# OmarZOS/deep-learning-at-scale

Measured on AMD Instinct MI355X. Metric: rows/sec (whole node), LSTM seq64 regression at 1/2/4/8 MI355X; val MSE parity, higher is better.
Workload: dtype bf16; 1 GPU; global_batch=8192, per_gpu_batch=8192, seq_len=64, parallelism=dp1

## Files before the change

deep-learning-at-scale_amd/csrc/binding.cpp:

```cpp
#include <torch/extension.h>
#include <ATen/hip/impl/HIPStreamMasqueradingAsCUDA.h>
#include <ATen/hip/impl/HIPGuardImplMasqueradingAsCUDA.h>

#include <cstdlib>
#include <map>
#include <type_traits>
#include <mutex>
#include <vector>

#include "kernels.h"

namespace {

using wf::bf16_t;

int diag_env(const char* name, int dflt) {
  if (wf::dbg_mask() != ~0) return dflt;
  const char* v = std::getenv(name);
  return v != nullptr ? std::atoi(v) : dflt;
}

bool disable_glds() {
  static const bool off = diag_env("WELLFLOW_NO_GLDS", 0) == 1;
  return off;
}

hipStream_t cur_stream() { return c10::hip::getCurrentHIPStreamMasqueradingAsCUDA().stream(); }

void check_t(const at::Tensor& t, at::ScalarType dt, const char* name) {
  TORCH_CHECK(t.defined(), name, ": undefined tensor");
  TORCH_CHECK(t.is_cuda(), name, ": must be a GPU tensor");
  TORCH_CHECK(t.scalar_type() == dt, name, ": expected dtype ", dt, " got ", t.scalar_type());
  TORCH_CHECK(t.is_contiguous(), name, ": must be contiguous");
  TORCH_CHECK(reinterpret_cast<uintptr_t>(t.data_ptr()) % 16 == 0, name,
              ": data pointer must be 16-byte aligned");
}

void check_extent(const at::Tensor& t, int64_t need, const char* name) {
  TORCH_CHECK(t.numel() >= need, name, ": needs at least ", need, " elements, has ", t.numel());
}

bf16_t* bfp(const at::Tensor& t) { return reinterpret_cast<bf16_t*>(t.data_ptr()); }
float* fp(const at::Tensor& t) { return t.data_ptr<float>(); }

template <class T>
T* opt_ptr(const c10::optional<at::Tensor>& t, at::ScalarType dt, const char* name,
           int64_t need) {
  if (!t.has_value() || !t->defined()) return nullptr;
  check_t(*t, dt, name);
  check_extent(*t, need, name);
  return reinterpret_cast<T*>(t->data_ptr());
}

int64_t operand_extent(bool mn, int64_t rows, int64_t K, int64_t ld) {
  if (rows == 0 || K == 0) return 0;
  return mn ? (K - 1) * ld + rows : (rows - 1) * ld + K;
}

void gemm(const at::Tensor& A, bool a_mn, int64_t lda, const at::Tensor& B, bool b_mn, int64_t ldb,
          int64_t M, int64_t N, int64_t K, int64_t ksplit, c10::optional<at::Tensor> outF,
          c10::optional<at::Tensor> outH, int64_t ldo, c10::optional<at::Tensor> bias,
          c10::optional<at::Tensor> mask, int64_t ldm, double mask_scale,
          c10::optional<at::Tensor> colsum, double alpha, double beta, int64_t act, bool atomic,
          double drop_p, int64_t seed, int64_t big_tile, c10::optional<at::Tensor> seed_dev) {
  TORCH_CHECK(wf::dw_tile_valid(big_tile), "gemm: tile ", big_tile, " does not exist; valid ids are 0 (128x128), ",
              "1 (256x128), 3 (256x192), 4 / 5 (256x192, 5- / 4-slot ring), 7 (best for N)");
  check_t(A, at::kBFloat16, "A");
  check_t(B, at::kBFloat16, "B");
  TORCH_CHECK(M > 0 && N > 0 && K > 0, "gemm: empty problem");
  TORCH_CHECK(lda % 8 == 0 && ldb % 8 == 0, "gemm: lda/ldb must be multiples of 8");
  TORCH_CHECK(a_mn ? (M % 8 == 0) : (K % 8 == 0), "gemm: A contiguous extent must be a multiple of 8");
  TORCH_CHECK(b_mn ? (N % 8 == 0) : (K % 8 == 0), "gemm: B contiguous extent must be a multiple of 8");
  TORCH_CHECK(a_mn ? lda >= M : lda >= K, "gemm: lda too small");
  TORCH_CHECK(b_mn ? ldb >= N : ldb >= K, "gemm: ldb too small");
  check_extent(A, operand_extent(a_mn, M, K, lda), "A");
  check_extent(B, operand_extent(b_mn, N, K, ldb), "B");
  TORCH_CHECK(ldo >= N, "gemm: ldo < N");
  const int64_t out_need = (M - 1) * ldo + N;
  wf::GemmEpilogue e;
  e.outF = opt_ptr<float>(outF, at::kFloat, "outF", out_need);
  e.outH = opt_ptr<bf16_t>(outH, at::kBFloat16, "outH", out_need);
  TORCH_CHECK(e.outF || e.outH, "gemm: need an output");
  TORCH_CHECK(!atomic || (e.outF && !e.outH && beta == 0.0), "gemm: atomic needs outF only, beta 0");
  TORCH_CHECK(beta == 0.0 || e.outF, "gemm: beta needs outF");
  e.ldo = ldo;
  e.bias = opt_ptr<float>(bias, at::kFloat, "bias", N);
  if (mask.has_value() && mask->defined()) TORCH_CHECK(ldm >= N, "gemm: ldm < N");
  e.mask = opt_ptr<bf16_t>(mask, at::kBFloat16, "mask", (M - 1) * ldm + N);
  e.ldm = ldm;
  e.mask_scale = (float)mask_scale;
  e.colsum = opt_ptr<float>(colsum, at::kFloat, "colsum", N);
  e.alpha = (float)alpha;
  e.beta = (float)beta;
  e.act = (int)act;
  e.atomic = atomic ? 1 : 0;
  e.drop_p = (float)drop_p;
  e.seed = (unsigned long long)seed;
  if (seed_dev.has_value() && seed_dev->defined()) {
    TORCH_CHECK(seed_dev->is_cuda() && seed_dev->scalar_type() == at::kLong && seed_dev->numel() >= 1,
                "gemm: seed_dev must be a GPU int64 tensor");
    e.seed_dev = reinterpret_cast<const long long*>(seed_dev->data_ptr<int64_t>());
  }
  e.big_tile = (int)big_tile;
  TORCH_CHECK(ksplit == 1 || atomic, "gemm: split-K needs atomic accumulation");
  e.stage_ok = (e.outH != nullptr && e.outF == nullptr && !atomic && beta == 0.0 && N % 8 == 0 &&
                ldo % 8 == 0 && (e.mask == nullptr || ldm % 8 == 0))
                   ? 1 : 0;
  const int64_t Mc = (M + 127) / 128 * 128, Nc = (N + 127) / 128 * 128;
  int64_t kchunk = (K + std::max<int64_t>(ksplit, 1) - 1) / std::max<int64_t>(ksplit, 1);
  kchunk = (kchunk + 63) / 64 * 64;
  const bool glds_ok = (K % 64 == 0) && (kchunk % 64 == 0) &&
                       A.numel() >= operand_extent(a_mn, Mc, K, lda) + (a_mn ? 0 : 0) &&
                       B.numel() >= operand_extent(b_mn, Nc, K, ldb) &&
                       (a_mn || Mc == M || lda >= K) && (b_mn || Nc == N || ldb >= K);
  const c10::hip::OptionalHIPGuardMasqueradingAsCUDA guard(A.device());
  wf::launch_gemm(bfp(A), lda, a_mn, bfp(B), ldb, b_mn, (int)M, (int)N, (int)K, (int)ksplit, e,
                  cur_stream(), glds_ok && !disable_glds());
}

wf::LstmDims lstm_dims(int64_t B, int64_t T, int64_t F, int64_t KX, int64_t H) {
  TORCH_CHECK(B > 0 && T > 0 && H > 0, "lstm: bad dims");
  TORCH_CHECK(H % 128 == 0, "lstm: hidden size must be a multiple of 128");
  TORCH_CHECK(KX % 64 == 0 && F + 1 <= KX, "lstm: KX must be a multiple of 64 and > F");
  wf::LstmDims d;
  d.B = (int)B; d.T = (int)T; d.F = (int)F; d.KX = (int)KX; d.H = (int)H;
  d.xcd_map = diag_env("WELLFLOW_XCD_MAP", 1) == 0 ? 0 : 1;
  d.nt = diag_env("WELLFLOW_NT", 1) == 0 ? 0 : 1;
  const char* pd = std::getenv("WELLFLOW_PF_DBG");
  d.dbg = (pd != nullptr ? std::atoi(pd) : 0) & wf::dbg_mask();
  const char* sl = std::getenv("WELLFLOW_SPIN_LIMIT");
  d.spin_limit = sl != nullptr ? (unsigned)std::strtoul(sl, nullptr, 10) : 0u;
  const char* ft = std::getenv("WELLFLOW_FORCE_TIMEOUT");
  if (ft != nullptr && ft[0] == '1') d.dbg |= 1 << 21;
  return d;
}

void check_lstm_state(const at::Tensor& XH, const at::Tensor& Cst, const at::Tensor& S,
                      const wf::LstmDims& d) {
  const int64_t KA = d.KX + d.H, G = 4 * d.H;
  const int64_t Bp = (d.B + 15) / 16 * 16;
  check_t(XH, at::kBFloat16, "XH");
  check_t(Cst, at::kBFloat16, "Cst");
  check_t(S, at::kBFloat16, "S");
  check_extent(XH, (int64_t)(d.T + 1) * d.B * KA, "XH");
  check_extent(Cst, (int64_t)(d.T + 1) * Bp * d.H, "Cst");
  check_extent(S, (int64_t)d.T * Bp * G, "S");
}

void lstm_pack_x(const at::Tensor& x, const at::Tensor& XH, int64_t B, int64_t T, int64_t F,
                 int64_t KX, int64_t H, bool full) {
  auto d = lstm_dims(B, T, F, KX, H);
  check_t(x, at::kFloat, "x");
  check_extent(x, B * T * F, "x");
  check_t(XH, at::kBFloat16, "XH");
  check_extent(XH, (T + 1) * B * (KX + H), "XH");
  const c10::hip::OptionalHIPGuardMasqueradingAsCUDA guard(x.device());
  wf::launch_lstm_pack_x(fp(x), bfp(XH), d, cur_stream(), full);
}

void lstm_pack_x_win(const at::Tensor& table, const at::Tensor& starts, const at::Tensor& idx, const at::Tensor& XH,
                     int64_t B, int64_t T, int64_t F, int64_t KX, int64_t H, bool full) {
  auto d = lstm_dims(B, T, F, KX, H);
  check_t(table, at::kFloat, "table");
  TORCH_CHECK(table.dim() == 2 && table.size(1) == F && table.size(0) >= T, "lstm_pack_x_win: table must be [>= T][F]");
  check_t(starts, at::kLong, "starts");
  check_t(idx, at::kLong, "idx");
  check_extent(idx, B, "idx");
  TORCH_CHECK(starts.numel() >= 1, "lstm_pack_x_win: no windows");
  check_t(XH, at::kBFloat16, "XH");
  check_extent(XH, (T + 1) * B * (KX + H), "XH");
  const c10::hip::OptionalHIPGuardMasqueradingAsCUDA guard(table.device());
  wf::launch_lstm_pack_x(fp(table), bfp(XH), d, cur_stream(), full, reinterpret_cast<const long*>(starts.data_ptr<int64_t>()),
                         reinterpret_cast<const long*>(idx.data_ptr<int64_t>()), starts.numel(), table.size(0));
}

void lstm_forward(const at::Tensor& XH, const at::Tensor& Wp, const at::Tensor& Cst,
                  const at::Tensor& S, const at::Tensor& cf32, int64_t B, int64_t T, int64_t F, int64_t KX,
                  int64_t H, int64_t variant) {
  auto d = lstm_dims(B, T, F, KX, H);
  d.fwd_variant = (int)variant;
  check_lstm_state(XH, Cst, S, d);
  check_t(Wp, at::kBFloat16, "Wp");
  check_extent(Wp, 4 * H * (KX + H), "Wp");
  check_t(cf32, at::kFloat, "cf32");
  check_extent(cf32, (B + 15) / 16 * 16 * H, "cf32");
  const c10::hip::OptionalHIPGuardMasqueradingAsCUDA guard(XH.device());
  auto s = cur_stream();
  for (int t = 0; t < d.T; ++t) wf::launch_lstm_fwd_step(t, bfp(XH), bfp(Wp), bfp(Cst), bfp(S), fp(cf32), d, s);
}

void check_sync(const at::Tensor& sync) {
  check_t(sync, at::kInt, "sync");
}

bool persistent_status(int st, const char* what) {
  TORCH_CHECK(st >= 0, what, ": launch failed: ", hipGetErrorString((hipError_t)(-st)));
  return st == 1;
}

bool lstm_forward_persistent(const at::Tensor& XH, const at::Tensor& Wp, const at::Tensor& Cst,
                             const at::Tensor& S, const at::Tensor& sync, int64_t B, int64_t T, int64_t F,
                             int64_t KX, int64_t H) {
  auto d = lstm_dims(B, T, F, KX, H);
  check_lstm_state(XH, Cst, S, d);
  check_t(Wp, at::kBFloat16, "Wp");
  check_extent(Wp, 4 * H * (KX + H), "Wp");
  check_sync(sync);
  const c10::hip::OptionalHIPGuardMasqueradingAsCUDA guard(XH.device());
  return persistent_status(wf::launch_lstm_fwd_persistent(bfp(XH), bfp(Wp), bfp(Cst), bfp(S),
                                                          reinterpret_cast<unsigned*>(sync.data_ptr<int>()),
                                                          sync.numel(), d, cur_stream()),
                           "persistent LSTM forward");
}

void check_lstm_bwd(const at::Tensor& WhhT, const at::Tensor& DG, const at::Tensor& dcarry, const at::Tensor& dy,
                    const at::Tensor& w_out, int64_t B, int64_t T, int64_t H) {
  check_t(WhhT, at::kBFloat16, "WhhT");
  check_extent(WhhT, H * 4 * H, "WhhT");
  check_t(DG, at::kBFloat16, "DG");
// ... 1246 lines not shown
```

deep-learning-at-scale_amd/csrc/gemm.hip:

```cpp
#include <cstdlib>

#include "gemm_core.h"
#include "kernels.h"

namespace wf {

__device__ __forceinline__ unsigned long long drop_seed(const GemmEpilogue& e) {
  return e.seed_dev != nullptr ? e.seed ^ ((unsigned long long)e.seed_dev[0] * 0xD1B54A32D192ED03ull) : e.seed;
}

template <int BM, int BN, int LA, int LB, int STAGES, int WM = 2, int WN = 2>
__global__ __launch_bounds__(64 * WM * WN) void gemm_kernel(const bf16_t* __restrict__ A, long lda,
                                                   const bf16_t* __restrict__ B, long ldb,
                                                   int M, int N, int K, int kchunk,
                                                   GemmEpilogue e) {
  using C = GemmCfg<BM, BN, LA, LB, WM, WN>;
  constexpr int LDSB = STAGES * C::STAGE > C::LDS_BYTES ? STAGES * C::STAGE : C::LDS_BYTES;
  __shared__ __attribute__((aligned(16))) char smem[LDSB];
  const int tiles_n = (N + BN - 1) / BN;
  const int tiles = ((M + BM - 1) / BM) * tiles_n;
  const int L = xcd_remap(blockIdx.x, gridDim.x);
  const int split = L / tiles, t = L % tiles;
  const int m0 = (t / tiles_n) * BM, n0 = (t % tiles_n) * BN;
  const int kbeg = split * kchunk;
// ... 23 lines not shown
        *reinterpret_cast<uint4*>(mt + chunk_off(row, c8)) = v;
      }
      __syncthreads();
    }
#pragma unroll
    for (int j = 0; j < C::TN; ++j) {
      const int n = cc.col(j);
      const int col = n - n0;
      const bool nok = n < N;
      const float bn = (e.bias != nullptr && nok) ? e.bias[n] : 0.f;
      float csum = 0.f;
#pragma unroll
      for (int i = 0; i < C::TM; ++i) {
#pragma unroll
        for (int r = 0; r < 4; ++r) {
          const int m = cc.row(i, r);
          const int row = m - m0;
          const int lo = chunk_off(row, col >> 3) + (col & 7);
          float v = e.alpha * acc[i][j][r] + bn;
          if (e.act == 1) v = fmaxf(v, 0.f);
          if (e.drop_p > 0.f)
            v = uniform_hash(drop_seed(e), (unsigned long long)m * N + n) >= e.drop_p
                    ? v * (1.f / (1.f - e.drop_p)) : 0.f;
          if (e.mask != nullptr) v = bf2f(mt[lo]) > 0.f ? v * e.mask_scale : 0.f;
          const bf16_t vb = f2bf(v);
          ot[lo] = vb;
          if (nok && m < M) csum += bf2f(vb);
        }
      }
      if (e.colsum != nullptr) {
        csum += __shfl_xor(csum, 16, 64);
        csum += __shfl_xor(csum, 32, 64);
        if ((threadIdx.x & 63) < 16 && nok) atomicAdd(e.colsum + n, csum);
      }
    }
    __syncthreads();
    for (int q = threadIdx.x; q < BM * CPR; q += C::NT) {
      const int row = q / CPR, c8 = q % CPR;
      const int m = m0 + row, n = n0 + c8 * 8;
      if (m < M && n < N)
        *reinterpret_cast<uint4*>(e.outH + (size_t)m * e.ldo + n) =
            *reinterpret_cast<const uint4*>(ot + chunk_off(row, c8));
    }
    return;
  }

#pragma unroll
  for (int j = 0; j < C::TN; ++j) {
    const int n = cc.col(j);
    const bool nok = n < N;
    const float bn = (e.bias != nullptr && nok) ? e.bias[n] : 0.f;
    float csum = 0.f;
#pragma unroll
    for (int i = 0; i < C::TM; ++i) {
#pragma unroll
      for (int r = 0; r < 4; ++r) {
        const int m = cc.row(i, r);
        if (!nok || m >= M) continue;
        float v = e.alpha * acc[i][j][r];
        const size_t o = (size_t)m * e.ldo + n;
        if (e.atomic) {
          atomicAdd(e.outF + o, v);
          continue;
        }
        if (e.beta != 0.f) v += e.beta * e.outF[o];
        v += bn;
        if (e.act == 1) v = fmaxf(v, 0.f);
        if (e.drop_p > 0.f)
          v = uniform_hash(drop_seed(e), (unsigned long long)m * N + n) >= e.drop_p
                  ? v * (1.f / (1.f - e.drop_p)) : 0.f;
        if (e.mask != nullptr)
          v = bf2f(e.mask[(size_t)m * e.ldm + n]) > 0.f ? v * e.mask_scale : 0.f;
        csum += v;
        if (e.outF != nullptr) e.outF[o] = v;
        if (e.outH != nullptr) e.outH[o] = f2bf(v);
      }
    }
    if (e.colsum != nullptr) {
      csum += __shfl_xor(csum, 16, 64);
      csum += __shfl_xor(csum, 32, 64);
      if ((threadIdx.x & 63) < 16 && nok) atomicAdd(e.colsum + n, csum);
    }
  }
}

template <int BM, int BN, int LA, int LB>
static void launch_cfg(const bf16_t* A, long lda, const bf16_t* B, long ldb, int M, int N, int K,
                       int ksplit, const GemmEpilogue& e, hipStream_t s, bool glds_ok) {
  const int tiles = ((M + BM - 1) / BM) * ((N + BN - 1) / BN);
  if (ksplit < 1) ksplit = 1;
  int kchunk = (K + ksplit - 1) / ksplit;
  kchunk = (kchunk + 63) / 64 * 64;
  if (kchunk < 64) kchunk = 64;
  const int nsplit = (K + kchunk - 1) / kchunk;
  const dim3 grid(tiles * (nsplit > 0 ? nsplit : 1));
  if (glds_ok && K % 64 == 0)
    hipLaunchKernelGGL((gemm_kernel<BM, BN, LA, LB, 3>), grid, dim3(256), 0, s, A, lda, B, ldb, M,
                       N, K, kchunk, e);
  else
    hipLaunchKernelGGL((gemm_kernel<BM, BN, LA, LB, 0>), grid, dim3(256), 0, s, A, lda, B, ldb, M,
                       N, K, kchunk, e);
}


static void launch_dw_big(const bf16_t* A, long lda, const bf16_t* B, long ldb, int M, int N, int K,
                          int ksplit, const GemmEpilogue& e, hipStream_t s) {
  constexpr int BM = 256, BN = 128;
  const int tiles = ((M + BM - 1) / BM) * ((N + BN - 1) / BN);
  int kchunk = ((K + ksplit - 1) / ksplit + 63) / 64 * 64;
  const int nsplit = (K + kchunk - 1) / kchunk;
  hipLaunchKernelGGL((gemm_kernel<BM, BN, MN_CONTIG, MN_CONTIG, 3, 4, 2>), dim3(tiles * nsplit),
                     dim3(512), 0, s, A, lda, B, ldb, M, N, K, kchunk, e);
}

template <int BM, int BN, int STAGES, int WM, int WN, int PRIO = 0>
__global__ __launch_bounds__(64 * WM * WN) void gemm_dw_kernel(const bf16_t* __restrict__ A, long lda,
                                                      const bf16_t* __restrict__ B, long ldb, int N,
                                                      int kchunk, int tiles, float* __restrict__ out,
                                                      long ldo, float alpha) {
  using C = GemmCfg<BM, BN, MN_CONTIG, MN_CONTIG, WM, WN>;
  __shared__ __attribute__((aligned(16))) char smem[STAGES * C::STAGE];
  const int tiles_n = N / BN;
  const int L = xcd_remap(blockIdx.x, gridDim.x);
  const int split = L / tiles, t = L % tiles;
  const int m0 = (t / tiles_n) * BM, n0 = (t % tiles_n) * BN;
  f32x4 acc[C::TM][C::TN];
  gemm_mainloop_glds2<C, STAGES, PRIO>(A, lda, B, ldb, split * kchunk, kchunk / 64, m0, n0, smem, acc);
  const AccCoord<C> cc(m0, n0);
#pragma unroll
  for (int j = 0; j < C::TN; ++j)
#pragma unroll
    for (int i = 0; i < C::TM; ++i)
#pragma unroll
      for (int r = 0; r < 4; ++r)
        atomicAdd(out + (size_t)cc.row(i, r) * ldo + cc.col(j), alpha * acc[i][j][r]);
}

static int equal_ksplit(int K, int ksplit) {
  int nsplit = ksplit;
  while (nsplit > 1 && K % (64 * nsplit) != 0) --nsplit;
  return nsplit;
}

static void launch_dw_192(const bf16_t* A, long lda, const bf16_t* B, long ldb, int M, int N, int K,
                          int ksplit, const GemmEpilogue& e, hipStream_t s) {
  constexpr int BM = 256, BN = 192;
  const int tiles = (M / BM) * (N / BN);
  const int nsplit = equal_ksplit(K, ksplit);
  const int kchunk = K / nsplit;
  hipLaunchKernelGGL((gemm_dw_kernel<BM, BN, 2, 4, 2, 1>), dim3(tiles * nsplit), dim3(512), 0, s, A, lda, B, ldb,
                     N, kchunk, tiles, e.outF, e.ldo, e.alpha);
}

template <int BM, int BN, int NSLOT, int WM, int WN, int PRIO, int BKD = 32>
__global__ __launch_bounds__(64 * WM * WN) void gemm_dw_h_kernel(const bf16_t* __restrict__ A, long lda,
                                                        const bf16_t* __restrict__ B, long ldb, int N,
                                                        int kchunk, int tiles, float* __restrict__ out,
                                                        long ldo, float alpha, float* __restrict__ slab,
                                                        long slab_stride) {
  using C = GemmCfg<BM, BN, MN_CONTIG, MN_CONTIG, WM, WN>;
  constexpr int STAGE = (BM + BN) * BKD * 2;
  __shared__ __attribute__((aligned(16))) char smem[NSLOT * STAGE];
  const int tiles_n = N / BN;
  const int L = xcd_remap(blockIdx.x, gridDim.x);
  const int split = L / tiles, t = L % tiles;
  const int m0 = (t / tiles_n) * BM, n0 = (t % tiles_n) * BN;
  f32x4 acc[C::TM][C::TN];
  gemm_mainloop_glds_h<C, NSLOT, PRIO, BKD>(A, lda, B, ldb, split * kchunk, kchunk / BKD, m0, n0, smem, acc);
  const AccCoord<C> cc(m0, n0);
  if (slab != nullptr) {
    float* o = slab + (size_t)split * slab_stride;
#pragma unroll
    for (int j = 0; j < C::TN; ++j)
#pragma unroll
      for (int i = 0; i < C::TM; ++i)
#pragma unroll
        for (int r = 0; r < 4; ++r) o[(size_t)cc.row(i, r) * ldo + cc.col(j)] = alpha * acc[i][j][r];
    return;
  }
#pragma unroll
  for (int j = 0; j < C::TN; ++j)
#pragma unroll
    for (int i = 0; i < C::TM; ++i)
#pragma unroll
      for (int r = 0; r < 4; ++r)
        atomicAdd(out + (size_t)cc.row(i, r) * ldo + cc.col(j), alpha * acc[i][j][r]);
}

static void launch_dw_192h(const bf16_t* A, long lda, const bf16_t* B, long ldb, int M, int N, int K,
                           int ksplit, int nslot, const GemmEpilogue& e, hipStream_t s) {
  constexpr int BM = 256, BN = 192;
  const int tiles = (M / BM) * (N / BN);
  const int nsplit = equal_ksplit(K, ksplit);
  const int kchunk = K / nsplit;
  const dim3 grid(tiles * nsplit);
  if (nslot == 5)
    hipLaunchKernelGGL((gemm_dw_h_kernel<BM, BN, 5, 4, 2, 1>), grid, dim3(512), 0, s, A, lda, B, ldb, N, kchunk,
                       tiles, e.outF, e.ldo, e.alpha, nullptr, 0L);
  else
    hipLaunchKernelGGL((gemm_dw_h_kernel<BM, BN, 4, 4, 2, 1>), grid, dim3(512), 0, s, A, lda, B, ldb, N, kchunk,
                       tiles, e.outF, e.ldo, e.alpha, nullptr, 0L);
}

__global__ __launch_bounds__(256) void dw_slab_reduce_kernel(float* __restrict__ out, const float* __restrict__ slab,
                                                             int nsplit, long n4) {
  const long i = (long)blockIdx.x * 256 + threadIdx.x;
  if (i >= n4) return;
  const float4* src = reinterpret_cast<const float4*>(slab) + i;
  float4 a = reinterpret_cast<float4*>(out)[i];
  for (int s0 = 0; s0 < nsplit; s0 += 8) {
    float4 v[8];
#pragma unroll
    for (int j = 0; j < 8; ++j) v[j] = s0 + j < nsplit ? src[(size_t)(s0 + j) * n4] : make_float4(0.f, 0.f, 0.f, 0.f);
#pragma unroll
    for (int j = 0; j < 8; ++j) {
      a.x += v[j].x;
      a.y += v[j].y;
      a.z += v[j].z;
      a.w += v[j].w;
    }
  }
  reinterpret_cast<float4*>(out)[i] = a;
}

static void launch_dw_288w(const bf16_t* A, long lda, const bf16_t* B, long ldb, int M, int N, int K,
                           int ksplit, const GemmEpilogue& e, hipStream_t s) {
  constexpr int BM = 256, BN = 288;
  const int tiles = (M / BM) * (N / BN);
  static const int cus = [] {
    int dev = 0, n = 0;
    if (hipGetDevice(&dev) != hipSuccess || hipDeviceGetAttribute(&n, hipDeviceAttributeMultiprocessorCount, dev) != hipSuccess)
      return 256;
    return n;
  }();
  if (ksplit * tiles > cus && cus / tiles >= 1) ksplit = cus / tiles;
  const int nsplit = equal_ksplit(K, ksplit);
  const int kchunk = K / nsplit;
  const long mn = (long)M * N;
  const bool use_slab = e.slab != nullptr && e.ldo == N && nsplit > 1 && (long)nsplit * mn <= e.slab_cap && mn % 4 == 0;
  hipLaunchKernelGGL((gemm_dw_h_kernel<BM, BN, 4, 4, 2, 1, 32>), dim3(tiles * nsplit), dim3(512), 0, s, A, lda, B,
                     ldb, N, kchunk, tiles, e.outF, e.ldo, e.alpha, use_slab ? e.slab : nullptr, use_slab ? mn : 0L);
  if (use_slab) {
    const long n4 = mn / 4;
    hipLaunchKernelGGL(dw_slab_reduce_kernel, dim3((unsigned)((n4 + 255) / 256)), dim3(256), 0, s, e.outF,
                       (const float*)e.slab, nsplit, n4);
  }
}

void launch_gemm(const bf16_t* A, long lda, int a_mn, const bf16_t* B, long ldb, int b_mn, int M,
                 int N, int K, int ksplit, const GemmEpilogue& e, hipStream_t s, bool glds_ok) {
  if (a_mn && b_mn && glds_ok && e.atomic && e.big_tile != kDwGeneric && M % 256 == 0 && K % 64 == 0) {
    const int ks = ksplit < 1 ? 1 : ksplit;
    if (e.big_tile == kDwBest && N % 288 == 0)
      launch_dw_288w(A, lda, B, ldb, M, N, K, ks, e, s);
    else if ((e.big_tile == kDw256x192Ring5 || e.big_tile == kDw256x192Ring4) && N % 192 == 0)
      launch_dw_192h(A, lda, B, ldb, M, N, K, ks, e.big_tile == kDw256x192Ring5 ? 5 : 4, e, s);
    else if (e.big_tile != kDw256x128 && N % 192 == 0)
      launch_dw_192(A, lda, B, ldb, M, N, K, ks, e, s);
    else
      launch_dw_big(A, lda, B, ldb, M, N, K, ks, e, s);
    return;
  }
  if (!a_mn && !b_mn)
    launch_cfg<128, 128, K_CONTIG, K_CONTIG>(A, lda, B, ldb, M, N, K, ksplit, e, s, glds_ok);
  else if (!a_mn && b_mn)
    launch_cfg<128, 128, K_CONTIG, MN_CONTIG>(A, lda, B, ldb, M, N, K, ksplit, e, s, glds_ok);
  else if (a_mn && !b_mn)
    launch_cfg<128, 128, MN_CONTIG, K_CONTIG>(A, lda, B, ldb, M, N, K, ksplit, e, s, glds_ok);
  else
    launch_cfg<128, 128, MN_CONTIG, MN_CONTIG>(A, lda, B, ldb, M, N, K, ksplit, e, s, glds_ok);
}

}
```

deep-learning-at-scale_amd/csrc/gemm_core.h:

```cpp
#pragma once
#include <type_traits>

#include "common.h"

namespace wf {

enum : int { K_CONTIG = 0, MN_CONTIG = 1 };

typedef __attribute__((address_space(3))) bf16x4 lds_bf16x4;

template <int R>
struct MnSwz {
  static constexpr int C = R / 16;
  static constexpr bool POW2 = (C & (C - 1)) == 0;
  static constexpr int RSH = C == 12 ? 1 : (C == 18 ? 2 : 0);
  __host__ __device__ static constexpr int hmask() { return POW2 ? C - 1 : 7; }
  __device__ static __forceinline__ int hk(int k) { return ((k & 3) | ((k >> 1) & 4)) & hmask(); }
  __device__ static __forceinline__ int pos(int j, int h) { return POW2 ? (j ^ h) : (j + (h >> RSH)) % C; }
  __device__ static __forceinline__ int data(int p, int h) { return POW2 ? (p ^ h) : (p + C - (h >> RSH)) % C; }
};

template <int R, int L, int NT_ = 256>
struct OpTile {
  static constexpr int NT = NT_;
// ... 248 lines not shown
      const int hk = (q | ((g & 1) << 2)) & MnSwz<R>::hmask();
#pragma unroll
      for (int i = 0; i < NB; ++i)
        fb[i] = (8 * g + q) * (R * 2) + (MnSwz<R>::pos((rw >> 4) + i, hk) << 5) + p * 8;
    }
  }

  template <int KK, int TOFF>
  __device__ __forceinline__ bf16x8 frag(const char* smem, int i) const {
    if constexpr (L == K_CONTIG) {
      return *reinterpret_cast<const bf16x8*>(smem + fb[KK] + TOFF + i * 16 * 128);
    } else {
      bf16x8 out;
#pragma unroll
      for (int h = 0; h < 2; ++h) {
        const char* a = smem + fb[i] + TOFF + (KK * 32 + 4 * h) * (R * 2);
        bf16x4 v = __builtin_amdgcn_ds_read_tr16_b64_v4i16((lds_bf16x4*)a);
        out[4 * h + 0] = v[0];
        out[4 * h + 1] = v[1];
        out[4 * h + 2] = v[2];
        out[4 * h + 3] = v[3];
      }
      return out;
    }
  }
};

template <class C, int STAGES, int PRIO = 0>
__device__ __forceinline__ void gemm_mainloop_glds2(const bf16_t* __restrict__ A, long lda,
                                                    const bf16_t* __restrict__ B, long ldb, int kbeg,
                                                    int nk, int m0, int n0, char* smem,
                                                    f32x4 (&acc)[C::TM][C::TN]) {
  static_assert(STAGES >= 2 && STAGES <= 6, "2..6 stages");
  using OA = GldsOperand<C::BM, C::LA_, C::NT>;
  using OB = GldsOperand<C::BN, C::LB_, C::NT>;
  constexpr int STAGE = OA::TILE_BYTES + OB::TILE_BYTES;
  constexpr int LPT = OA::Q::PER_WAVE + OB::Q::PER_WAVE;
  const int lane = threadIdx.x & 63;
  const int wid = __builtin_amdgcn_readfirstlane(threadIdx.x >> 6);
  const int wm = wid / C::WN, wn = wid % C::WN;
#pragma unroll
  for (int i = 0; i < C::TM; ++i)
#pragma unroll
    for (int j = 0; j < C::TN; ++j) acc[i][j] = f32x4{0.f, 0.f, 0.f, 0.f};
  if (nk <= 0) return;
  OA oa;
  OB ob;
  oa.init(A, lda, m0, kbeg, wid, lane);
  ob.init(B, ldb, n0, kbeg, wid, lane);
  FragReader<C::BM, C::LA_, C::WTM> fa;
  FragReader<C::BN, C::LB_, C::WTN> fbr;
  fa.init(wm * C::WTM, lane);
  fbr.init(wn * C::WTN, lane);

#pragma unroll
  for (int s = 0; s < STAGES - 1; ++s) {
    if (s < nk) {
      oa.issue(s, smem + s * STAGE, wid);
      ob.issue(s, smem + s * STAGE + OA::TILE_BYTES, wid);
    }
  }

  auto body = [&](int tt, auto uc) {
    constexpr int u = decltype(uc)::value;
    const int ahead = min(nk - 1, tt + STAGES - 2) - tt;
    if constexpr (STAGES >= 5) {
      if (ahead >= STAGES - 2) wait_vmcnt<(STAGES - 2) * LPT>();
      else if (ahead == 3) wait_vmcnt<3 * LPT>();
      else if (ahead == 2) wait_vmcnt<2 * LPT>();
      else if (ahead == 1) wait_vmcnt<LPT>();
      else wait_vmcnt<0>();
    } else if constexpr (STAGES >= 4) {
      if (ahead >= 2) wait_vmcnt<2 * LPT>();
      else if (ahead == 1) wait_vmcnt<LPT>();
      else wait_vmcnt<0>();
    } else if constexpr (STAGES == 3) {
      if (ahead >= 1) wait_vmcnt<LPT>();
      else wait_vmcnt<0>();
    } else {
      wait_vmcnt<0>();
    }
    __builtin_amdgcn_s_barrier();
    asm volatile("" ::: "memory");
    const int tn = tt + STAGES - 1;
    if (tn < nk) {
      constexpr int sn = (u + STAGES - 1) % STAGES;
      oa.issue(tn, smem + sn * STAGE, wid);
      ob.issue(tn, smem + sn * STAGE + OA::TILE_BYTES, wid);
    }
    static_for<0, 2>([&](auto kc) {
      constexpr int KK = decltype(kc)::value;
      bf16x8 a[C::TM], b[C::TN];
#pragma unroll
      for (int i = 0; i < C::TM; ++i) a[i] = fa.template frag<KK, u * STAGE>(smem, i);
#pragma unroll
      for (int j = 0; j < C::TN; ++j) b[j] = fbr.template frag<KK, u * STAGE + OA::TILE_BYTES>(smem, j);
      if constexpr (PRIO == 1) __builtin_amdgcn_s_setprio(1);
#pragma unroll
      for (int i = 0; i < C::TM; ++i)
#pragma unroll
        for (int j = 0; j < C::TN; ++j)
          acc[i][j] = __builtin_amdgcn_mfma_f32_16x16x32_bf16(a[i], b[j], acc[i][j], 0, 0, 0);
      if constexpr (PRIO == 1) __builtin_amdgcn_s_setprio(0);
    });
  };

  int t = 0;
  for (; t + STAGES <= nk; t += STAGES)
    static_for<0, STAGES>([&](auto uc) { body(t + decltype(uc)::value, uc); });
  static_for<0, STAGES>([&](auto uc) {
    if (t + decltype(uc)::value < nk) body(t + decltype(uc)::value, uc);
  });
  __builtin_amdgcn_s_barrier();
  asm volatile("" ::: "memory");
}

template <int R, int L, int NT, int BKD>
struct GldsOpH {
  static_assert(L == MN_CONTIG, "half-step ring: MN-contiguous operands only");
  static constexpr int BYTES = R * BKD * 2;
  static constexpr int PIECES = BYTES / 1024;
  static constexpr int NW = NT / 64;
  static constexpr int MAXPW = (PIECES + NW - 1) / NW;
  static constexpr int REM = PIECES % NW;
  static_assert(BYTES % 1024 == 0 && PIECES >= NW, "tile image must be whole 1-KiB pieces, >= 1 per wave");
  using SW = MnSwz<R>;
  unsigned src[MAXPW];
  __amdgpu_buffer_rsrc_t rsrc;
  int kstep_bytes;

  __device__ __forceinline__ void init(const bf16_t* p, long ld, int row0, int kbeg, int wid, int lane) {
#pragma unroll
    for (int i = 0; i < MAXPW; ++i) {
      const int o = (i * NW + wid) * 1024 + lane * 16;
      const int k = o / (R * 2), b = o % (R * 2);
      const int col = (SW::data(b >> 5, SW::hk(k)) << 4) + (((b >> 4) & 1) << 3);
      src[i] = (unsigned)(((long)k * ld + col) * 2);
    }
    rsrc = __builtin_amdgcn_make_buffer_rsrc(const_cast<bf16_t*>(p + (size_t)kbeg * ld + row0), 0, 0x7FFFFFFF,
                                             0x00020000);
    kstep_bytes = (int)(BKD * ld * 2);
  }
  __device__ __forceinline__ void issue(int step, char* lds_tile, int wid) const {
    const int so = step * kstep_bytes;
#pragma unroll
    for (int i = 0; i < MAXPW; ++i) {
      if (i + 1 < MAXPW || REM == 0 || wid < REM)
        __builtin_amdgcn_raw_ptr_buffer_load_lds(rsrc, (lds_void*)(lds_tile + (i * NW + wid) * 1024), 16, (int)src[i],
                                                 so, 0, 0);
    }
  }
};

template <class C, int NSLOT, int PRIO = 0, int BKD = 32>
__device__ __forceinline__ void gemm_mainloop_glds_h(const bf16_t* __restrict__ A, long lda,
                                                     const bf16_t* __restrict__ B, long ldb, int kbeg,
                                                     int nh, int m0, int n0, char* smem,
                                                     f32x4 (&acc)[C::TM][C::TN]) {
  static_assert(BKD == 32 || BKD == 64, "32- or 64-deep steps");
  static_assert(NSLOT >= 2 && NSLOT <= 6, "2..6 slots");
  using OA = GldsOpH<C::BM, C::LA_, C::NT, BKD>;
  using OB = GldsOpH<C::BN, C::LB_, C::NT, BKD>;
  static_assert(OA::REM == 0 || OB::REM == 0, "at most one operand with an uneven piece split");
  constexpr int STAGE = OA::BYTES + OB::BYTES;
  constexpr int LHI = OA::MAXPW + OB::MAXPW;
  constexpr int LLO = LHI - ((OA::REM | OB::REM) != 0 ? 1 : 0);
  constexpr int NHI = OA::REM ? OA::REM : (OB::REM ? OB::REM : C::NT / 64);
  const int lane = threadIdx.x & 63;
  const int wid = __builtin_amdgcn_readfirstlane(threadIdx.x >> 6);
  const int wm = wid / C::WN, wn = wid % C::WN;
  const bool hi = wid < NHI;
#pragma unroll
  for (int i = 0; i < C::TM; ++i)
#pragma unroll
    for (int j = 0; j < C::TN; ++j) acc[i][j] = f32x4{0.f, 0.f, 0.f, 0.f};
  if (nh <= 0) return;
  OA oa;
  OB ob;
  oa.init(A, lda, m0, kbeg, wid, lane);
  ob.init(B, ldb, n0, kbeg, wid, lane);
  FragReader<C::BM, C::LA_, C::WTM> fa;
  FragReader<C::BN, C::LB_, C::WTN> fbr;
  fa.init(wm * C::WTM, lane);
  fbr.init(wn * C::WTN, lane);

#pragma unroll
  for (int s = 0; s < NSLOT - 1; ++s) {
    if (s < nh) {
      oa.issue(s, smem + s * STAGE, wid);
      ob.issue(s, smem + s * STAGE + OA::BYTES, wid);
    }
  }
  auto body = [&](int tt, auto uc) {
    constexpr int u = decltype(uc)::value;
    const int ahead = min(nh - 1, tt + NSLOT - 2) - tt;
    __builtin_amdgcn_sched_barrier(0);
    static_for<0, NSLOT - 1>([&](auto ac) {
      constexpr int a = NSLOT - 2 - decltype(ac)::value;
      if (ahead == a) {
        if (hi) wait_vmcnt<a * LHI>();
        else wait_vmcnt<a * LLO>();
      }
    });
    __builtin_amdgcn_s_barrier();
    asm volatile("" ::: "memory");
    const int tn = tt + NSLOT - 1;
    if (tn < nh) {
      constexpr int sn = (u + NSLOT - 1) % NSLOT;
      oa.issue(tn, smem + sn * STAGE, wid);
      ob.issue(tn, smem + sn * STAGE + OA::BYTES, wid);
    }
    int so = u * STAGE;
    asm volatile("" : "+v"(so));
    const char* sl = smem + so;
    static_for<0, BKD / 32>([&](auto kc) {
      constexpr int KK = decltype(kc)::value;
      bf16x8 a[C::TM], b[C::TN];
#pragma unroll
      for (int i = 0; i < C::TM; ++i) a[i] = fa.template frag<KK, 0>(sl, i);
#pragma unroll
      for (int j = 0; j < C::TN; ++j) b[j] = fbr.template frag<KK, OA::BYTES>(sl, j);
      if constexpr (PRIO == 1) __builtin_amdgcn_s_setprio(1);
#pragma unroll
      for (int i = 0; i < C::TM; ++i)
#pragma unroll
        for (int j = 0; j < C::TN; ++j)
          acc[i][j] = __builtin_amdgcn_mfma_f32_16x16x32_bf16(a[i], b[j], acc[i][j], 0, 0, 0);
      if constexpr (PRIO == 1) __builtin_amdgcn_s_setprio(0);
    });
  };
  int t = 0;
  for (; t + NSLOT <= nh; t += NSLOT)
    static_for<0, NSLOT>([&](auto uc) { body(t + decltype(uc)::value, uc); });
  static_for<0, NSLOT>([&](auto uc) {
    if (t + decltype(uc)::value < nh) body(t + decltype(uc)::value, uc);
  });
  __builtin_amdgcn_s_barrier();
  asm volatile("" ::: "memory");
}

template <class C>
struct AccCoord {
  int mb, nb;
  __device__ __forceinline__ AccCoord(int m0, int n0) {
    const int wid = threadIdx.x >> 6;
    mb = m0 + (wid / C::WN) * C::WTM;
    nb = n0 + (wid % C::WN) * C::WTN;
  }
  __device__ __forceinline__ int row(int i, int r) const {
    return mb + i * 16 + 4 * ((threadIdx.x & 63) >> 4) + r;
  }
  __device__ __forceinline__ int col(int j) const { return nb + j * 16 + (threadIdx.x & 15); }
};

}
```

deep-learning-at-scale_amd/csrc/kernels.h:

```cpp
#pragma once
#include <hip/hip_runtime.h>
#include <stdint.h>

namespace wf {

typedef unsigned short bf16_t;

enum DwTile : int {
  kDwGeneric = 0,
  kDw256x128 = 1,
  kDw256x192 = 3,
  kDw256x192Ring5 = 4,
  kDw256x192Ring4 = 5,
  kDwBest = 7,
};
inline bool dw_tile_valid(long t) {
  return t == kDwGeneric || t == kDw256x128 || t == kDw256x192 || t == kDw256x192Ring5 || t == kDw256x192Ring4 ||
         t == kDwBest;
}

struct GemmEpilogue {
  float* outF = nullptr;
  bf16_t* outH = nullptr;
  long ldo = 0;
  const float* bias = nullptr;
  const bf16_t* mask = nullptr;
  long ldm = 0;
  float mask_scale = 1.f;
  float* colsum = nullptr;
  float alpha = 1.f, beta = 0.f;
  int act = 0;
  int atomic = 0;
  float drop_p = 0.f;
  unsigned long long seed = 0;
  const long long* seed_dev = nullptr;
  int stage_ok = 0;
  int big_tile = kDwGeneric;
  float* slab = nullptr;
  long slab_cap = 0;
};

void launch_gemm(const bf16_t* A, long lda, int a_mn, const bf16_t* B, long ldb, int b_mn, int M,
                 int N, int K, int ksplit, const GemmEpilogue& e, hipStream_t s,
                 bool glds_ok = false);

struct LstmDims {
  int B, T, F, KX, H;
  int fwd_variant = 0;
  int bwd_variant = 0;
  int xcd_map = 1;
  int nt = 1;
  int dbg = 0;
  int row_off = 0;
  unsigned spin_limit = 0;
};
int dbg_mask();
void launch_lstm_pack_x(const float* x, bf16_t* XH, LstmDims d, hipStream_t s, bool full = true,
                        const long* starts = nullptr, const long* idx = nullptr, long nwin = 0, long nrows = 0);
void launch_lstm_fwd_step(int t, bf16_t* XH, const bf16_t* Wp, bf16_t* Cst, bf16_t* S, float* cf32,
                          LstmDims d, hipStream_t s);
int lstm_persistent_sync_words(int row_blocks);
long lstm_persistent_sync_total(int row_blocks);
int launch_lstm_fwd_persistent(bf16_t* XH, const bf16_t* Wp, bf16_t* Cst, bf16_t* S, unsigned* sync,
                                long sync_words, LstmDims d, hipStream_t s);
int launch_lstm_bwd_persistent(const bf16_t* WhhT, const bf16_t* Cst, const bf16_t* S, bf16_t* DG,
                                const float* dcarry, unsigned* sync, long sync_words, LstmDims d,
                                hipStream_t s);
void launch_lstm_bwd_step(int t, const bf16_t* WhhT, const bf16_t* Cst, const bf16_t* S,
                          bf16_t* DG, float* dcarry, const float* dy, const float* w_out,
                          LstmDims d, hipStream_t s);
void launch_lstm_pack_weights(const float* W, bf16_t* Wp, bf16_t* WhhT, LstmDims d,
                              hipStream_t s);

bool launch_mlp2_fwd(const bf16_t* X, int Fp, const bf16_t* W1, const float* b1, const bf16_t* W2, const float* b2,
                     const float* w3, const float* b3, const float* y, bf16_t* H1, bf16_t* H2, unsigned* M2,
                     float* dw3, float* db3, float* pred, float* dy, float* loss_sum, float dy_scale, int B,
                     const long long* rows, long nrows, hipStream_t s, float* red = nullptr);
bool launch_mlp2_bwd(const bf16_t* H1, const bf16_t* H2, const unsigned* M2, const float* dy, const float* w3, const bf16_t* W2,
                     const bf16_t* X, int Fp, bf16_t* dZ1, bf16_t* dZ2, float* dW1, float* db1, float* db2,
                     float* dw3, float* db3, int B, const bf16_t* W1, const float* b1, const long long* rows,
                     long nrows, hipStream_t s, float* red = nullptr);
bool launch_mlp2_dw2(const bf16_t* dZ2, const bf16_t* X, int Fp, const long long* rows, long nrows, const bf16_t* W1,
                     const float* b1, int B, int nsplit, float* dW2, hipStream_t s, float* red = nullptr);
constexpr int kMlpRedCopies = 64, kMlpRedCopies2 = 4, kMlpRedRow = 9216;
constexpr int kMlpRedLoss = 0, kMlpRedDb3 = 1, kMlpRedDw3 = 2, kMlpRedDb1 = 258, kMlpRedDb2 = 514, kMlpRedDW1 = 770;
constexpr int kMlpRedSlabRows = 256, kMlpRedSlabRow = 256 * 64;
constexpr long kMlpRedSlabOff = (long)kMlpRedCopies * kMlpRedRow + (long)kMlpRedCopies2 * 65536;
constexpr int kMlpRedSlab2Rows = 256;
constexpr long kMlpRedSlab2Off = kMlpRedSlabOff + (long)kMlpRedSlabRows * kMlpRedSlabRow;
constexpr long kMlpRedFloats = kMlpRedSlab2Off + (long)kMlpRedSlab2Rows * 65536;
int mlp2_train_grid(int B);
constexpr int kMlpSmallScratch = 49728 + 65536;
struct MlpSmallArgs {
  const bf16_t* X;
  const float* Y;
  const long long* rows;
  long nrows;
  int Fp, B, K;
  float* p;
  float* m;
  float* v;
  float* step;
  float lr, b1, b2, eps, wd, dy_scale, clip;
  bf16_t* shadow;
  bf16_t* w2t;
  float* loss_acc;
  float* scr;
  unsigned* sync;
  unsigned spin_limit;
  long oW1, ob1, oW2, ob2, ow3, ob3;
  unsigned long long* stamps;
};
bool launch_mlp_small(const MlpSmallArgs& a, hipStream_t s);
constexpr int kCnnSmallScratch = 2 * 28 * 64 * 16 * 2 + 2 * 64 * 16 * 2;
struct CnnSmallArgs {
  const float* X;
  const float* Y;
  const long long* rows;
  long nrows;
  int B, K, O, taps, filters, drop, loss_kind;
  float keep_scale, clip, scale;
  unsigned seed;
  long long* rng;
  float* p;
  float* vel;
  float* step;
  float lr, decay, momentum, gscale;
  int nesterov;
  float* loss_acc;
  float* scr;
  unsigned* sync;
  unsigned spin_limit;
  unsigned long long* stamps;
};
bool launch_cnn_small(const CnnSmallArgs& a, hipStream_t s);
bool mlp_bwd8();
void launch_mlp2_reduce(float* red, int Fp, int B, float* loss_sum, float* db3, float* dw3, float* db1, float* db2,
                        float* dW1, float* dW2, hipStream_t s, int dw2_rows = 0);
bool launch_mlp2_step(const bf16_t* X, int Fp, const bf16_t* W1, const float* b1, const bf16_t* W2, const float* b2,
                      const float* w3, const float* b3, const float* y, float dy_scale, int B, const long long* rows,
                      long nrows, bf16_t* dZ2, float* pred, float* red, bool dz_frag, hipStream_t s,
                      const bf16_t* W2T = nullptr, float clip = 0.f);
int launch_mlp2_dw2f(const bf16_t* dZ2F, const bf16_t* X, int Fp, const long long* rows, long nrows, const bf16_t* W1,
                     const float* b1, int B, int nsplit, float* red, hipStream_t s);

struct CnnDims {
  int L, C, taps, T, Fp, Kc, O;
  float drop_p;
};
bool cnn_fused_supported(const CnnDims& d);
int cnn_fwd_grid(int B);
int cnn_bwd_chunks(int B);
long cnn_part_floats(int B, const CnnDims& d, long* wd, long* wc, long* f);
void launch_cnn_sgd_pack(float* p, float* g, float* vel, long n, float* step, float lr, float decay, float momentum,
                         int nesterov, float gscale, int zero_g, const CnnDims& d, bf16_t* WcA, bf16_t* WdF,
                         bf16_t* WdB, hipStream_t s, const float* clip = nullptr, float clipvalue = 0.f);
void launch_cnn_pack(const float* Wc, const float* Wd, const CnnDims& d, bf16_t* WcA, bf16_t* WdF, bf16_t* WdB,
                     hipStream_t s);
void launch_cnn_forward(const float* x, int B, const CnnDims& d, const bf16_t* WcA, const bf16_t* WdF,
                        const float* bd, const float* y, float* dout, float* pred, float* part, int train,
                        int loss_kind, float clip, float scale, unsigned seed, const long long* rng, hipStream_t s);
void launch_cnn_backward(const float* x, int B, const CnnDims& d, const bf16_t* WcA, const bf16_t* WdB,
                         const float* dout, unsigned seed, const long long* rng, float* part_wd, float* part_wc,
                         hipStream_t s);
void launch_cnn_reduce(const float* part_wd, const float* part_wc, const float* part_f, int B, const CnnDims& d,
                       float* gWc, float* gWd, float* gbd, float* loss_sum, long long* rng, hipStream_t s);

void launch_head_fwd(const bf16_t* Hm, long ldh, int B, int Hd, const float* w, const float* b0,
                     const float* target, float* pred, float* dy, float* loss_sum, float dy_scale,
                     hipStream_t s);
bool launch_head_fwd_bwd(const bf16_t* Hm, long ldh, int B, int Hd, const float* w, const float* b0,
// ... 78 lines not shown
```

Baseline: 2.041 million rows/s.

## Stagger half the waves in the dW GEMM mainloop to overlap MFMA with LDS reads

Rewrites the glds_h GEMM mainloop so waves 4-7 of a 512-thread workgroup run one interval behind waves 0-3. The late group issues its MFMAs on the previous fragments right after the barrier, then loads the next fragments. This is meant to spread LDS reads and matrix-core work across the two wave groups instead of having all waves contend in lockstep. The old lockstep behaviour stays available as tile id 13, the 64-deep step option is dropped, and register pressure goes up because fragments are held across iterations.

```diff
diff --git a/deep-learning-at-scale_amd/csrc/binding.cpp b/deep-learning-at-scale_amd/csrc/binding.cpp
--- a/deep-learning-at-scale_amd/csrc/binding.cpp
+++ b/deep-learning-at-scale_amd/csrc/binding.cpp
@@ -64,7 +64,7 @@
           c10::optional<at::Tensor> colsum, double alpha, double beta, int64_t act, bool atomic,
           double drop_p, int64_t seed, int64_t big_tile, c10::optional<at::Tensor> seed_dev) {
   TORCH_CHECK(wf::dw_tile_valid(big_tile), "gemm: tile ", big_tile, " does not exist; valid ids are 0 (128x128), ",
-              "1 (256x128), 3 (256x192), 4 / 5 (256x192, 5- / 4-slot ring), 7 (best for N)");
+              "1 (256x128), 3 (256x192), 4 / 5 (256x192, 5- / 4-slot ring), 7 (best for N), 13 (7 without the wave stagger)");
   check_t(A, at::kBFloat16, "A");
   check_t(B, at::kBFloat16, "B");
   TORCH_CHECK(M > 0 && N > 0 && K > 0, "gemm: empty problem");
diff --git a/deep-learning-at-scale_amd/csrc/gemm.hip b/deep-learning-at-scale_amd/csrc/gemm.hip
--- a/deep-learning-at-scale_amd/csrc/gemm.hip
+++ b/deep-learning-at-scale_amd/csrc/gemm.hip
@@ -199,7 +199,7 @@
                      N, kchunk, tiles, e.outF, e.ldo, e.alpha);
 }
 
-template <int BM, int BN, int NSLOT, int WM, int WN, int PRIO, int BKD = 32>
+template <int BM, int BN, int NSLOT, int WM, int WN, int PRIO, int BKD = 32, bool STAGGER = true>
 __global__ __launch_bounds__(64 * WM * WN) void gemm_dw_h_kernel(const bf16_t* __restrict__ A, long lda,
                                                         const bf16_t* __restrict__ B, long ldb, int N,
                                                         int kchunk, int tiles, float* __restrict__ out,
@@ -213,7 +213,7 @@
   const int split = L / tiles, t = L % tiles;
   const int m0 = (t / tiles_n) * BM, n0 = (t % tiles_n) * BN;
   f32x4 acc[C::TM][C::TN];
-  gemm_mainloop_glds_h<C, NSLOT, PRIO, BKD>(A, lda, B, ldb, split * kchunk, kchunk / BKD, m0, n0, smem, acc);
+  gemm_mainloop_glds_h<C, NSLOT, PRIO, BKD, STAGGER>(A, lda, B, ldb, split * kchunk, kchunk / BKD, m0, n0, smem, acc);
   const AccCoord<C> cc(m0, n0);
   if (slab != nullptr) {
     float* o = slab + (size_t)split * slab_stride;
@@ -271,7 +271,7 @@
 }
 
 static void launch_dw_288w(const bf16_t* A, long lda, const bf16_t* B, long ldb, int M, int N, int K,
-                           int ksplit, const GemmEpilogue& e, hipStream_t s) {
+                           int ksplit, bool stagger, const GemmEpilogue& e, hipStream_t s) {
   constexpr int BM = 256, BN = 288;
   const int tiles = (M / BM) * (N / BN);
   static const int cus = [] {
@@ -285,8 +285,14 @@
   const int kchunk = K / nsplit;
   const long mn = (long)M * N;
   const bool use_slab = e.slab != nullptr && e.ldo == N && nsplit > 1 && (long)nsplit * mn <= e.slab_cap && mn % 4 == 0;
-  hipLaunchKernelGGL((gemm_dw_h_kernel<BM, BN, 4, 4, 2, 1, 32>), dim3(tiles * nsplit), dim3(512), 0, s, A, lda, B,
-                     ldb, N, kchunk, tiles, e.outF, e.ldo, e.alpha, use_slab ? e.slab : nullptr, use_slab ? mn : 0L);
+  if (stagger)
+    hipLaunchKernelGGL((gemm_dw_h_kernel<BM, BN, 4, 4, 2, 1, 32, true>), dim3(tiles * nsplit), dim3(512), 0, s, A, lda,
+                       B, ldb, N, kchunk, tiles, e.outF, e.ldo, e.alpha, use_slab ? e.slab : nullptr,
+                       use_slab ? mn : 0L);
+  else
+    hipLaunchKernelGGL((gemm_dw_h_kernel<BM, BN, 4, 4, 2, 1, 32, false>), dim3(tiles * nsplit), dim3(512), 0, s, A,
+                       lda, B, ldb, N, kchunk, tiles, e.outF, e.ldo, e.alpha, use_slab ? e.slab : nullptr,
+                       use_slab ? mn : 0L);
   if (use_slab) {
     const long n4 = mn / 4;
     hipLaunchKernelGGL(dw_slab_reduce_kernel, dim3((unsigned)((n4 + 255) / 256)), dim3(256), 0, s, e.outF,
@@ -298,8 +304,8 @@
                  int N, int K, int ksplit, const GemmEpilogue& e, hipStream_t s, bool glds_ok) {
   if (a_mn && b_mn && glds_ok && e.atomic && e.big_tile != kDwGeneric && M % 256 == 0 && K % 64 == 0) {
     const int ks = ksplit < 1 ? 1 : ksplit;
-    if (e.big_tile == kDwBest && N % 288 == 0)
-      launch_dw_288w(A, lda, B, ldb, M, N, K, ks, e, s);
+    if ((e.big_tile == kDwBest || e.big_tile == kDw256x288Lockstep) && N % 288 == 0)
+      launch_dw_288w(A, lda, B, ldb, M, N, K, ks, e.big_tile == kDwBest, e, s);
     else if ((e.big_tile == kDw256x192Ring5 || e.big_tile == kDw256x192Ring4) && N % 192 == 0)
       launch_dw_192h(A, lda, B, ldb, M, N, K, ks, e.big_tile == kDw256x192Ring5 ? 5 : 4, e, s);
     else if (e.big_tile != kDw256x128 && N % 192 == 0)
diff --git a/deep-learning-at-scale_amd/csrc/gemm_core.h b/deep-learning-at-scale_amd/csrc/gemm_core.h
--- a/deep-learning-at-scale_amd/csrc/gemm_core.h
+++ b/deep-learning-at-scale_amd/csrc/gemm_core.h
@@ -424,20 +424,23 @@
   }
 };
 
-template <class C, int NSLOT, int PRIO = 0, int BKD = 32>
+template <class C, int NSLOT, int PRIO = 0, int BKD = 32, bool STAGGER = true>
 __device__ __forceinline__ void gemm_mainloop_glds_h(const bf16_t* __restrict__ A, long lda,
                                                      const bf16_t* __restrict__ B, long ldb, int kbeg,
                                                      int nh, int m0, int n0, char* smem,
                                                      f32x4 (&acc)[C::TM][C::TN]) {
-  static_assert(BKD == 32 || BKD == 64, "32- or 64-deep steps");
+  static_assert(BKD == 32, "32-deep steps");
   static_assert(NSLOT >= 2 && NSLOT <= 6, "2..6 slots");
   using OA = GldsOpH<C::BM, C::LA_, C::NT, BKD>;
   using OB = GldsOpH<C::BN, C::LB_, C::NT, BKD>;
   static_assert(OA::REM == 0 || OB::REM == 0, "at most one operand with an uneven piece split");
+  constexpr int NW = C::NT / 64;
   constexpr int STAGE = OA::BYTES + OB::BYTES;
   constexpr int LHI = OA::MAXPW + OB::MAXPW;
   constexpr int LLO = LHI - ((OA::REM | OB::REM) != 0 ? 1 : 0);
-  constexpr int NHI = OA::REM ? OA::REM : (OB::REM ? OB::REM : C::NT / 64);
+  constexpr int NHI = OA::REM ? OA::REM : (OB::REM ? OB::REM : NW);
+  static_assert(!STAGGER || NW == 8, "the stagger pairs waves w and w + 4 of a 512-thread workgroup");
+  static_assert(!STAGGER || LHI == LLO || NHI <= NW / 2, "extra pieces must stay in the early group");
   const int lane = threadIdx.x & 63;
   const int wid = __builtin_amdgcn_readfirstlane(threadIdx.x >> 6);
   const int wm = wid / C::WN, wn = wid % C::WN;
@@ -463,35 +466,19 @@
       ob.issue(s, smem + s * STAGE + OA::BYTES, wid);
     }
   }
-  auto body = [&](int tt, auto uc) {
-    constexpr int u = decltype(uc)::value;
-    const int ahead = min(nh - 1, tt + NSLOT - 2) - tt;
-    __builtin_amdgcn_sched_barrier(0);
-    static_for<0, NSLOT - 1>([&](auto ac) {
-      constexpr int a = NSLOT - 2 - decltype(ac)::value;
-      if (ahead == a) {
-        if (hi) wait_vmcnt<a * LHI>();
-        else wait_vmcnt<a * LLO>();
-      }
-    });
-    __builtin_amdgcn_s_barrier();
-    asm volatile("" ::: "memory");
-    const int tn = tt + NSLOT - 1;
-    if (tn < nh) {
-      constexpr int sn = (u + NSLOT - 1) % NSLOT;
-      oa.issue(tn, smem + sn * STAGE, wid);
-      ob.issue(tn, smem + sn * STAGE + OA::BYTES, wid);
-    }
-    int so = u * STAGE;
-    asm volatile("" : "+v"(so));
-    const char* sl = smem + so;
-    static_for<0, BKD / 32>([&](auto kc) {
-      constexpr int KK = decltype(kc)::value;
-      bf16x8 a[C::TM], b[C::TN];
-#pragma unroll
-      for (int i = 0; i < C::TM; ++i) a[i] = fa.template frag<KK, 0>(sl, i);
-#pragma unroll
-      for (int j = 0; j < C::TN; ++j) b[j] = fbr.template frag<KK, OA::BYTES>(sl, j);
+
+  auto ring = [&](auto late_c) {
+    constexpr bool LATE = decltype(late_c)::value;
+    bf16x8 a[C::TM], b[C::TN];
+    if constexpr (LATE) {
+#pragma unroll
+      for (int i = 0; i < C::TM; ++i) a[i] = bf16x8{0, 0, 0, 0, 0, 0, 0, 0};
+#pragma unroll
+      for (int j = 0; j < C::TN; ++j) b[j] = bf16x8{0, 0, 0, 0, 0, 0, 0, 0};
+    }
+    int cur = 0, prev = (NSLOT - 1) * STAGE;
+
+    auto mfma = [&]() {
       if constexpr (PRIO == 1) __builtin_amdgcn_s_setprio(1);
 #pragma unroll
       for (int i = 0; i < C::TM; ++i)
@@ -499,16 +486,59 @@
         for (int j = 0; j < C::TN; ++j)
           acc[i][j] = __builtin_amdgcn_mfma_f32_16x16x32_bf16(a[i], b[j], acc[i][j], 0, 0, 0);
       if constexpr (PRIO == 1) __builtin_amdgcn_s_setprio(0);
+    };
+    auto interval = [&](int tt, auto ahead_c, auto issue_c) {
+      constexpr int AHEAD = decltype(ahead_c)::value;
+      constexpr bool ISSUE = decltype(issue_c)::value;
+      __builtin_amdgcn_sched_barrier(0);
+      if constexpr (LATE || LHI == LLO || (STAGGER && NHI == NW / 2)) {
+        wait_vmcnt<AHEAD * (LATE ? LLO : LHI)>();
+      } else {
+        if (hi) wait_vmcnt<AHEAD * LHI>();
+        else wait_vmcnt<AHEAD * LLO>();
+      }
+      __builtin_amdgcn_s_barrier();
+      asm volatile("" ::: "memory");
+      if constexpr (LATE) {
+        mfma();
+        __builtin_amdgcn_sched_barrier(0);
+      }
+      if constexpr (ISSUE) {
+        oa.issue(tt + NSLOT - 1, smem + prev, wid);
+        ob.issue(tt + NSLOT - 1, smem + prev + OA::BYTES, wid);
+      }
+      if constexpr (LATE) __builtin_amdgcn_sched_barrier(0);
+      int so = cur;
+      asm volatile("" : "+v"(so));
+      const char* sl = smem + so;
+#pragma unroll
+      for (int i = 0; i < C::TM; ++i) a[i] = fa.template frag<0, 0>(sl, i);
+#pragma unroll
+      for (int j = 0; j < C::TN; ++j) b[j] = fbr.template frag<0, OA::BYTES>(sl, j);
+      if constexpr (LATE) {
+        __builtin_amdgcn_s_waitcnt(0xC07F);
+      } else {
+        mfma();
+      }
+      prev = cur;
+      cur = cur + STAGE == NSLOT * STAGE ? 0 : cur + STAGE;
+    };
+
+    int tt = 0;
+#pragma unroll 1
+    for (; tt + NSLOT <= nh; ++tt)
+      interval(tt, std::integral_constant<int, NSLOT - 2>{}, std::true_type{});
+    static_for<0, NSLOT - 1>([&](auto rc) {
+      constexpr int r = NSLOT - 2 - decltype(rc)::value;
+      if (r < nh) interval(nh - 1 - r, std::integral_constant<int, r>{}, std::false_type{});
     });
+    __builtin_amdgcn_sched_barrier(0);
+    __builtin_amdgcn_s_barrier();
+    asm volatile("" ::: "memory");
+    if constexpr (LATE) mfma();
   };
-  int t = 0;
-  for (; t + NSLOT <= nh; t += NSLOT)
-    static_for<0, NSLOT>([&](auto uc) { body(t + decltype(uc)::value, uc); });
-  static_for<0, NSLOT>([&](auto uc) {
-    if (t + decltype(uc)::value < nh) body(t + decltype(uc)::value, uc);
-  });
-  __builtin_amdgcn_s_barrier();
-  asm volatile("" ::: "memory");
+  if (STAGGER && wid >= NW / 2) ring(std::true_type{});
+  else ring(std::false_type{});
 }
 
 template <class C>
diff --git a/deep-learning-at-scale_amd/csrc/kernels.h b/deep-learning-at-scale_amd/csrc/kernels.h
--- a/deep-learning-at-scale_amd/csrc/kernels.h
+++ b/deep-learning-at-scale_amd/csrc/kernels.h
@@ -13,10 +13,11 @@
   kDw256x192Ring5 = 4,
   kDw256x192Ring4 = 5,
   kDwBest = 7,
+  kDw256x288Lockstep = 13,
 };
 inline bool dw_tile_valid(long t) {
   return t == kDwGeneric || t == kDw256x128 || t == kDw256x192 || t == kDw256x192Ring5 || t == kDw256x192Ring4 ||
-         t == kDwBest;
+         t == kDwBest || t == kDw256x288Lockstep;
 }
 
 struct GemmEpilogue {
```

Result: no change. 2.061 million rows/s, median of 2 (+1.0%).
